# aszepieniec/stark-brainfuck

Measured on AMD Instinct MI355X. Metric: goldilocks_ntt_field_elements_per_sec, higher is better.
Workload: dtype u64 (mod 2^64-2^32+1)

## Files before the change

stark_brainfuck_amd/csrc/air.hip:

```cpp
#include <algorithm>
#include <cstddef>
#include <vector>

#include "air_eval.hpp"
#include "lazy.hpp"
#include "runtime.hpp"

namespace bfs {

struct RandomizerValues {
    u64 v[64];
};

__global__ void __launch_bounds__(256) poly_evaluate_partial_kernel(const u64* coeffs, u64 stride, u64 h, u64 point, u64* partial, u32 first) {
    __shared__ u64 part[256];
    const u64* f = coeffs + (u64)(first + blockIdx.y) * stride;
    const u32 t = threadIdx.x;
    const u64 T = (u64)gridDim.x * 256, g = (u64)blockIdx.x * 256 + t;
    u64 acc = 0;
    if (g < h) {
        const u64 step = gl_pow(point, T);
        u64 k = g + (h - 1 - g) / T * T;
        for (;; k -= T) {
            acc = gl_add(gl_mul(acc, step), f[k]);
// ... 26 lines not shown
    __shared__ u64 part[256];
    const u64* f = coeffs + (u64)blockIdx.y * stride;
    u64 acc = 0;
    for (u64 j = (u64)blockIdx.x * 256 + threadIdx.x; j < len; j += (u64)gridDim.x * 256)
        if (f[j] != 0) acc |= j ? (j & (0 - j)) : (1ull << 63);
    part[threadIdx.x] = acc;
    __syncthreads();
    for (u32 s = 128; s > 0; s >>= 1) {
        if (threadIdx.x < s) part[threadIdx.x] |= part[threadIdx.x + s];
        __syncthreads();
    }
    if (threadIdx.x == 0 && part[0]) atomicOr((unsigned long long*)(out + blockIdx.y), (unsigned long long)part[0]);
}

struct AirArgs {
    const u64* base;
    const u64* ext;
    u64* out;
    u64 n;
    u64 first, count;
    u64 unit_distance;
    u64 height;
    u32 log_height;
    u64 omicron_inv;
    u64 offset;
    const u64* w_lo;
    const u64* w_hi;
    u32 lo_bits;
    Xfe ch[11];
    Xfe tm[5];
    Xfe pr[1];
};

struct LdsNextBase {
    const u64* p;
    __device__ __forceinline__ u64 operator[](int k) const { return p[k * 256]; }
};
struct LdsNextExt {
    const u64* p;
    __device__ __forceinline__ Xfe operator[](int k) const { return Xfe{{p[(3 * k) * 256], p[(3 * k + 1) * 256], p[(3 * k + 2) * 256]}}; }
};

struct Zerofiers {
    u64 boundary, transition, terminal;
    __device__ __forceinline__ Zerofiers(const AirArgs& a, u64 x) {
        const u64 za = gl_sub(x, 1), xo = gl_sub(x, a.omicron_inv);
        u64 zc = 1;
        if (a.height != 0) {
            u64 xh = x;
            for (u32 s = 0; s < a.log_height; ++s) xh = gl_sqr(xh);
            zc = gl_sub(xh, 1);
        }
        const u64 ab = gl_mul(za, xo);
        const u64 iabc = gl_inv(gl_mul(ab, zc));
        const u64 iab = gl_mul(iabc, zc);
        boundary = gl_mul(iab, xo);
        terminal = gl_mul(iab, za);
        transition = a.height != 0 ? gl_mul(xo, gl_mul(iabc, ab)) : 0;
    }
    __device__ __forceinline__ Zerofiers(const AirArgs& a, u64 x, u64 inv_x_minus_1, u64 inv_x_minus_omicron_inv, u64 inv_xh_minus_1) {
        boundary = inv_x_minus_1;
        terminal = inv_x_minus_omicron_inv;
        transition = a.height != 0 ? gl_mul(gl_sub(x, a.omicron_inv), inv_xh_minus_1) : 0;
    }
    template <int TABLE, int Q>
    __device__ __forceinline__ u64 of() const {
        typedef AirShape<TABLE> S;
        return Q < S::NB ? boundary : (Q < S::NB + S::NT ? transition : terminal);
    }
};

template <int TABLE>
struct QuotientStore {
    u64* out;
    u64 n, i;
    Zerofiers z;
    template <int Q> __device__ __forceinline__ void put(const Xfe& v) {
// ... 94 lines not shown
    static constexpr int kind(int k) { return k < NC ? 0 : (k - NC < S::NB ? 1 : (k - NC < S::NB + S::NT ? 2 : 3)); }
    static constexpr bool continues_run(int k) {
        if (k == 0 || kind(k) != kind(k - 1)) return false;
        return kind(k) == 0 ? true : q_degree(k - NC) == q_degree(k - 1 - NC);
    }
    static constexpr int words(int k) { return 2 * (is_ext(k) ? LAZY_W_EXT : LAZY_W_BASE); }
    static constexpr int offset(int k) {
        int o = 0;
        for (int j = 0; j < k; ++j) o += words(j);
        return o;
    }
    static constexpr int NW = offset(NTERM);
};

template <int TABLE>
struct CombineTerms {
    u64 w[CombineLayout<TABLE>::NW];
    u32 shift[(CombineLayout<TABLE>::NTERM + 1) & ~1];
};

template <int TABLE>
struct AirCombineArgs {
    AirArgs a;
    const u64* randomizer;
    Xfe w0;
    u64* acc;
    const u64 *inv_boundary, *inv_terminal, *inv_transition;
    CombineTerms<TABLE> terms;
};

template <int TABLE, bool GROUPED>
struct CombineSink {
    typedef CombineLayout<TABLE> Lay;
    const AirArgs& a;
    const CombineTerms<TABLE>& T;
    u64 i;
    Zerofiers z;
    Xfe acc;
    LazyX sa, sb;

    __device__ __forceinline__ u64 omega_pow(int k) const {
        return tw_pow(a.w_lo, a.w_hi, a.lo_bits, (i * T.shift[k]) & (a.n - 1));
    }
    template <int K> __device__ __forceinline__ void close_run() {
        lazyx_mac_scale(sa, lazyx_reduce(sb), omega_pow(K));
        sb = lazyx_zero();
    }
    template <int KIND> __device__ __forceinline__ void close_kind() {
        const Xfe kind_sum = lazyx_reduce(sa);
        sa = lazyx_zero();
        if constexpr (KIND == 0) acc = xfe_add(acc, kind_sum);
        else acc = xfe_add(acc, xfe_scale(kind_sum, KIND == 1 ? z.boundary : (KIND == 2 ? z.transition : z.terminal)));
    }
    template <int K> __device__ __forceinline__ void open() {
        if constexpr (K > 0) {
            constexpr bool new_kind = Lay::kind(K) != Lay::kind(K - 1);
            if constexpr (new_kind || !GROUPED || !Lay::continues_run(K)) close_run<K - 1>();
            if constexpr (new_kind) close_kind<Lay::kind(K - 1)>();
        }
    }
    template <int K> __device__ __forceinline__ void term_base(u64 v) {
        static_assert(!Lay::is_ext(K), "layout and generated code disagree");
        open<K>();
        lazyx_mac_base(sa, T.w + Lay::offset(K), v);
        lazyx_mac_base(sb, T.w + Lay::offset(K) + LAZY_W_BASE, v);
    }
    template <int K> __device__ __forceinline__ void term_ext(const Xfe& v) {
        static_assert(Lay::is_ext(K), "layout and generated code disagree");
        open<K>();
        lazyx_mac_ext(sa, T.w + Lay::offset(K), v);
        lazyx_mac_ext(sb, T.w + Lay::offset(K) + LAZY_W_EXT, v);
    }
    __device__ __forceinline__ void finish() {
        close_run<Lay::NTERM - 1>();
        close_kind<Lay::kind(Lay::NTERM - 1)>();
    }
    template <int Q> __device__ __forceinline__ void put(const Xfe& v) { term_ext<Lay::NC + Q>(v); }
    template <int Q> __device__ __forceinline__ void put_base(u64 v) { term_base<Lay::NC + Q>(v); }
};

template <int TABLE, int C, class Sink>
__device__ __forceinline__ void combine_columns(Sink& sink, const u64* bc, const Xfe* xc) {
    typedef AirShape<TABLE> S;
    if constexpr (C < S::BW) { sink.template term_base<C>(bc[C]); combine_columns<TABLE, C + 1>(sink, bc, xc); }
    else if constexpr (C < S::BW + S::XW) { sink.template term_ext<C>(xc[C - S::BW]); combine_columns<TABLE, C + 1>(sink, bc, xc); }
}

#ifndef BFS_COMBINE_WAVES
#define BFS_COMBINE_WAVES 3, 3, 4, 4, 4
#endif
#ifndef BFS_COMBINE_LDS_NEXT
#define BFS_COMBINE_LDS_NEXT 1
#endif
constexpr int combine_waves(int table) {
    constexpr int w[5] = {BFS_COMBINE_WAVES};
    return w[table];
}
template <int TABLE, bool GROUPED>
__global__ void __launch_bounds__(256, combine_waves(TABLE)) air_combine_kernel(const AirCombineArgs<TABLE> A) {
    typedef AirShape<TABLE> S;
    __shared__ CombineTerms<TABLE> T;
    {
        const u64* karg = (const u64*)__builtin_amdgcn_kernarg_segment_ptr();
        constexpr u32 first = offsetof(AirCombineArgs<TABLE>, terms) / 8, words = sizeof(CombineTerms<TABLE>) / 8;
        static_assert(offsetof(AirCombineArgs<TABLE>, terms) % 8 == 0 && sizeof(CombineTerms<TABLE>) % 8 == 0, "staged as 64-bit words");
        u64* dst = reinterpret_cast<u64*>(&T);
        for (u32 k = threadIdx.x; k < words; k += 256) dst[k] = karg[first + k];
    }
    __syncthreads();
    const AirArgs& a = A.a;
    const u64 i = a.first + (u64)blockIdx.x * blockDim.x + threadIdx.x;
    if (i < a.first + a.count) {
        u64 j = i + a.unit_distance;
        if (j >= a.n) j -= a.n;
        constexpr bool LDS_NEXT = ((BFS_COMBINE_LDS_NEXT) >> TABLE) & 1;
        __shared__ u64 next_row[LDS_NEXT ? (S::BW + 3 * S::XW) * 256 : 1];
        u64 bc[S::BW], bn[LDS_NEXT ? 1 : S::BW];
        Xfe xc[S::XW], xn[LDS_NEXT ? 1 : S::XW];
#pragma unroll
        for (int c = 0; c < S::BW; ++c) {
            bc[c] = a.base[(u64)c * a.n + i];
            if constexpr (LDS_NEXT) next_row[c * 256 + threadIdx.x] = a.base[(u64)c * a.n + j];
            else bn[c] = a.base[(u64)c * a.n + j];
        }
#pragma unroll
        for (int c = 0; c < S::XW; ++c)
#pragma unroll
            for (int l = 0; l < 3; ++l) {
                xc[c].c[l] = a.ext[(u64)(3 * c + l) * a.n + i];
                if constexpr (LDS_NEXT) next_row[(S::BW + 3 * c + l) * 256 + threadIdx.x] = a.ext[(u64)(3 * c + l) * a.n + j];
                else xn[c].c[l] = a.ext[(u64)(3 * c + l) * a.n + j];
            }
        Xfe acc;
        if (A.randomizer) acc = xfe_mul(A.w0, Xfe{{A.randomizer[i], A.randomizer[a.n + i], A.randomizer[2 * a.n + i]}});
        else acc = Xfe{{A.acc[i], A.acc[a.n + i], A.acc[2 * a.n + i]}};
        const u64 x = gl_mul(a.offset, tw_pow(a.w_lo, a.w_hi, a.lo_bits, i));
        CombineSink<TABLE, GROUPED> sink{a, T, i,
                                         A.inv_boundary ? Zerofiers(a, x, A.inv_boundary[i], A.inv_terminal[i], a.height != 0 ? A.inv_transition[i] : 0)
                                                        : Zerofiers(a, x),
                                         acc, lazyx_zero(), lazyx_zero()};
        combine_columns<TABLE, 0>(sink, bc, xc);
        if constexpr (LDS_NEXT) air_eval<TABLE>(bc, LdsNextBase{next_row + threadIdx.x}, xc, LdsNextExt{next_row + S::BW * 256 + threadIdx.x}, a, sink);
        else air_eval<TABLE>(bc, (const u64*)bn, xc, (const Xfe*)xn, a, sink);
        sink.finish();
        A.acc[i] = sink.acc.c[0];
        A.acc[a.n + i] = sink.acc.c[1];
        A.acc[2 * a.n + i] = sink.acc.c[2];
    }
}

__global__ void difference_combine_kernel(const u64* lhs, const u64* rhs, u64* acc, u64 n, u64 offset, const u64* w_lo, const u64* w_hi,
                                          u32 lo_bits, CombW w, const u64* inv_x_minus_1, u64 first, u64 count) {
    for (u64 i = first + (u64)blockIdx.x * blockDim.x + threadIdx.x; i < first + count; i += (u64)gridDim.x * blockDim.x) {
        const u64 z = inv_x_minus_1 ? inv_x_minus_1[i] : gl_inv(gl_sub(gl_mul(offset, tw_pow(w_lo, w_hi, lo_bits, i)), 1));
        const u64 xs = gl_mul(w.offset_pow, tw_pow(w_lo, w_hi, lo_bits, (i * w.shift) & (n - 1)));
        const Xfe weight = xfe_add(w.wa, xfe_scale(w.wb, xs));
        Xfe q;
#pragma unroll
        for (int l = 0; l < 3; ++l) q.c[l] = gl_mul(gl_sub(lhs[(u64)l * n + i], rhs[(u64)l * n + i]), z);
        const Xfe r = xfe_add(Xfe{{acc[i], acc[n + i], acc[2 * n + i]}}, xfe_mul(weight, q));
        acc[i] = r.c[0];
        acc[n + i] = r.c[1];
        acc[2 * n + i] = r.c[2];
    }
}

__global__ void difference_quotient_kernel(const u64* lhs, const u64* rhs, u64* out, u64 n, u64 offset, const u64* w_lo, const u64* w_hi, u32 lo_bits) {
    for (u64 i = (u64)blockIdx.x * blockDim.x + threadIdx.x; i < n; i += (u64)gridDim.x * blockDim.x) {
        const u64 x = gl_mul(offset, tw_pow(w_lo, w_hi, lo_bits, i));
        const u64 z = gl_inv(gl_sub(x, 1));
#pragma unroll
        for (int l = 0; l < 3; ++l) out[(u64)l * n + i] = gl_mul(gl_sub(lhs[(u64)l * n + i], rhs[(u64)l * n + i]), z);
    }
}

struct CombSrc {
    const u64* ptr;
    u32 is_ext, pad;
    u64 shift;
    Xfe wa, wb;
// ... 346 lines not shown
```

stark_brainfuck_amd/csrc/air_eval.hpp:

```cpp
#pragma once
#include "air_generated.hpp"

namespace bfs {

template <int TABLE> struct AirShape;
template <> struct AirShape<0> { static constexpr int BW = airgen::PROCESSOR_BASE_WIDTH, XW = airgen::PROCESSOR_EXT_WIDTH, NB = airgen::PROCESSOR_NUM_BOUNDARY, NT = airgen::PROCESSOR_NUM_TRANSITION, NZ = airgen::PROCESSOR_NUM_TERMINAL; };
template <> struct AirShape<1> { static constexpr int BW = airgen::INSTRUCTION_BASE_WIDTH, XW = airgen::INSTRUCTION_EXT_WIDTH, NB = airgen::INSTRUCTION_NUM_BOUNDARY, NT = airgen::INSTRUCTION_NUM_TRANSITION, NZ = airgen::INSTRUCTION_NUM_TERMINAL; };
template <> struct AirShape<2> { static constexpr int BW = airgen::MEMORY_BASE_WIDTH, XW = airgen::MEMORY_EXT_WIDTH, NB = airgen::MEMORY_NUM_BOUNDARY, NT = airgen::MEMORY_NUM_TRANSITION, NZ = airgen::MEMORY_NUM_TERMINAL; };
template <> struct AirShape<3> { static constexpr int BW = airgen::INPUT_BASE_WIDTH, XW = airgen::INPUT_EXT_WIDTH, NB = airgen::INPUT_NUM_BOUNDARY, NT = airgen::INPUT_NUM_TRANSITION, NZ = airgen::INPUT_NUM_TERMINAL; };
template <> struct AirShape<4> { static constexpr int BW = airgen::OUTPUT_BASE_WIDTH, XW = airgen::OUTPUT_EXT_WIDTH, NB = airgen::OUTPUT_NUM_BOUNDARY, NT = airgen::OUTPUT_NUM_TRANSITION, NZ = airgen::OUTPUT_NUM_TERMINAL; };

template <int TABLE, class Sink, class BN, class XN, class Args>
__device__ __forceinline__ void air_eval(const u64* bc, BN bn, const Xfe* xc, XN xn, const Args& a, Sink& sink) {
    if constexpr (TABLE == 0) airgen::air_processor(bc, bn, xc, xn, a.ch, a.tm, a.pr, sink);
    else if constexpr (TABLE == 1) airgen::air_instruction(bc, bn, xc, xn, a.ch, a.tm, a.pr, sink);
    else if constexpr (TABLE == 2) airgen::air_memory(bc, bn, xc, xn, a.ch, a.tm, a.pr, sink);
    else if constexpr (TABLE == 3) airgen::air_input(bc, bn, xc, xn, a.ch, a.tm, a.pr, sink);
    else airgen::air_output(bc, bn, xc, xn, a.ch, a.tm, a.pr, sink);
}

}
```

stark_brainfuck_amd/csrc/air_generated.hpp:

```cpp
#pragma once
#include "gl.hpp"

namespace bfs {
namespace airgen {

struct ArraySink {
    Xfe* out;
    template <int I> BFS_HD void put(const Xfe& v) { out[I] = v; }
    template <int I> BFS_HD void put_base(u64 v) { out[I] = xfe_lift(v); }
};

constexpr int PROCESSOR_BASE_WIDTH = 7, PROCESSOR_EXT_WIDTH = 4, PROCESSOR_NUM_BOUNDARY = 7, PROCESSOR_NUM_TRANSITION = 10, PROCESSOR_NUM_TERMINAL = 4;
constexpr bool PROCESSOR_Q_EXT[] = {false, false, false, false, false, true, true, false, false, false, false, false, false, true, true, true, true, true, true, true, true};
constexpr unsigned char PROCESSOR_Q_DEGREE[] = {1, 1, 1, 1, 1, 1, 1, 11, 9, 9, 1, 3, 3, 9, 9, 9, 9, 1, 9, 1, 1};
template <class Sink, class BN = const u64*, class XN = const Xfe*>
BFS_HD void air_processor(const u64* bc, BN bn, const Xfe* xc, XN xn, const Xfe* ch, const Xfe* tm, const Xfe* pr, Sink& sink) {
    sink.template put_base<0>(bc[0]);
    sink.template put_base<1>(bc[1]);
    sink.template put_base<2>(bc[4]);
    sink.template put_base<3>(bc[5]);
    sink.template put_base<4>(bc[6]);
    sink.template put<5>(xc[2]);
    sink.template put<6>(xc[3]);
    const u64 t0 = gl_sub(bc[2], 93ULL);
    const u64 t1 = gl_sub(bc[2], 60ULL);
    const u64 t2 = gl_mul(t0, t1);
    const u64 t3 = gl_sub(bc[2], 62ULL);
    const u64 t4 = gl_mul(t2, t3);
    const u64 t5 = gl_sub(bc[2], 44ULL);
    const u64 t6 = gl_mul(t4, t5);
    const u64 t7 = gl_sub(bc[2], 46ULL);
    const u64 t8 = gl_mul(t6, t7);
    const u64 t9 = gl_sub(bc[2], 43ULL);
    const u64 t10 = gl_mul(t8, t9);
    const u64 t11 = gl_sub(bc[2], 45ULL);
    const u64 t12 = gl_mul(t10, t11);
    const u64 t13 = gl_sub(bn[1], bc[1]);
    const u64 t14 = gl_sub(t13, 2ULL);
    const u64 t15 = gl_mul(bc[5], t14);
    const u64 t16 = gl_mul(bc[5], bc[6]);
    const u64 t17 = gl_sub(t16, 1ULL);
    const u64 t18 = gl_sub(bn[1], bc[3]);
    const u64 t19 = gl_mul(t17, t18);
    const u64 t20 = gl_add(t15, t19);
    const u64 t21 = gl_mul(t20, bc[2]);
    const u64 t22 = gl_mul(t12, t21);
    const u64 t23 = gl_sub(bc[2], 91ULL);
// ... 127 lines not shown
    const Xfe t143 = xfe_scale(t142, bc[2]);
    const Xfe t144 = xfe_sub(xn[2], xc[2]);
    const u64 t145 = gl_sub(44ULL, bc[2]);
    const Xfe t146 = xfe_scale(t144, t145);
    const Xfe t147 = xfe_add(t143, t146);
    sink.template put<15>(t147);
    const Xfe t148 = xfe_mul(xc[3], ch[9]);
    const Xfe t149 = xfe_sub(xn[3], t148);
    const Xfe t150 = xfe_sub_base(t149, bc[5]);
    const Xfe t151 = xfe_scale(t150, t68);
    const Xfe t152 = xfe_scale(t151, bc[2]);
    const Xfe t153 = xfe_sub(xn[3], xc[3]);
    const u64 t154 = gl_sub(46ULL, bc[2]);
    const Xfe t155 = xfe_scale(t153, t154);
    const Xfe t156 = xfe_add(t152, t155);
    sink.template put<16>(t156);
    const Xfe t157 = xfe_sub(tm[0], xc[0]);
    sink.template put<17>(t157);
    const Xfe t158 = xfe_sub(tm[1], t133);
    const Xfe t159 = xfe_scale(t158, bc[2]);
    const Xfe t160 = xfe_sub(tm[1], xc[1]);
    const Xfe t161 = xfe_scale(t160, t123);
    const Xfe t162 = xfe_add(t159, t161);
    sink.template put<18>(t162);
    const Xfe t163 = xfe_sub(tm[2], xc[2]);
    sink.template put<19>(t163);
    const Xfe t164 = xfe_sub(tm[3], xc[3]);
    sink.template put<20>(t164);
}
BFS_HD void air_processor_values(const u64* bc, const u64* bn, const Xfe* xc, const Xfe* xn, const Xfe* ch, const Xfe* tm, const Xfe* pr, Xfe* out) {
    ArraySink sink{out};
    air_processor(bc, bn, xc, xn, ch, tm, pr, sink);
}

constexpr int INSTRUCTION_BASE_WIDTH = 3, INSTRUCTION_EXT_WIDTH = 2, INSTRUCTION_NUM_BOUNDARY = 2, INSTRUCTION_NUM_TRANSITION = 6, INSTRUCTION_NUM_TERMINAL = 2;
constexpr bool INSTRUCTION_Q_EXT[] = {false, true, false, false, false, false, true, true, true, true};
constexpr unsigned char INSTRUCTION_Q_DEGREE[] = {1, 1, 2, 2, 2, 2, 9, 2, 1, 1};
template <class Sink, class BN = const u64*, class XN = const Xfe*>
BFS_HD void air_instruction(const u64* bc, BN bn, const Xfe* xc, XN xn, const Xfe* ch, const Xfe* tm, const Xfe* pr, Sink& sink) {
    sink.template put_base<0>(bc[0]);
    const Xfe t0 = xfe_scale(ch[0], bc[0]);
    const Xfe t1 = xfe_sub(xc[1], t0);
    const Xfe t2 = xfe_scale(ch[1], bc[1]);
    const Xfe t3 = xfe_sub(t1, t2);
    const Xfe t4 = xfe_scale(ch[2], bc[2]);
    const Xfe t5 = xfe_sub(t3, t4);
    sink.template put<1>(t5);
    const u64 t6 = gl_sub(bn[0], bc[0]);
    const u64 t7 = gl_sub(t6, 1ULL);
    const u64 t8 = gl_mul(t7, t6);
    sink.template put_base<2>(t8);
    const u64 t9 = gl_sub(bc[2], bn[1]);
    const u64 t10 = gl_mul(t6, t9);
    sink.template put_base<3>(t10);
    const u64 t11 = gl_sub(bn[1], bc[1]);
    const u64 t12 = gl_mul(t7, t11);
    sink.template put_base<4>(t12);
    const u64 t13 = gl_sub(bn[2], bc[2]);
    const u64 t14 = gl_mul(t7, t13);
    sink.template put_base<5>(t14);
    const Xfe t15 = xfe_scale(ch[0], bn[0]);
    const Xfe t16 = xfe_sub(ch[6], t15);
    const Xfe t17 = xfe_scale(ch[1], bn[1]);
    const Xfe t18 = xfe_sub(t16, t17);
    const Xfe t19 = xfe_scale(ch[2], bn[2]);
    const Xfe t20 = xfe_sub(t18, t19);
    const Xfe t21 = xfe_mul(xc[0], t20);
    const Xfe t22 = xfe_sub(t21, xn[0]);
    const Xfe t23 = xfe_scale(t22, bc[1]);
    const u64 t24 = gl_add(bc[0], 1ULL);
// ... 10 lines not shown
    const u64 t35 = gl_mul(t33, t34);
    const u64 t36 = gl_sub(bc[1], 45ULL);
    const u64 t37 = gl_mul(t35, t36);
    const u64 t38 = gl_sub(bc[1], 44ULL);
    const u64 t39 = gl_mul(t37, t38);
    const u64 t40 = gl_sub(bc[1], 46ULL);
    const u64 t41 = gl_mul(t39, t40);
    const Xfe t42 = xfe_sub(xc[0], xn[0]);
    const Xfe t43 = xfe_scale(t42, t41);
    const Xfe t44 = xfe_add(t26, t43);
    const u64 t45 = gl_sub(bc[0], bn[0]);
    const Xfe t46 = xfe_scale(t42, t45);
    const Xfe t47 = xfe_add(t44, t46);
    sink.template put<6>(t47);
    const Xfe t48 = xfe_mul(xc[1], ch[10]);
    const Xfe t49 = xfe_add(t48, t15);
    const Xfe t50 = xfe_add(t49, t17);
    const Xfe t51 = xfe_add(t50, t19);
    const Xfe t52 = xfe_sub(t51, xn[1]);
    const Xfe t53 = xfe_scale(t52, t6);
    const Xfe t54 = xfe_sub(xc[1], xn[1]);
    const Xfe t55 = xfe_scale(t54, t7);
    const Xfe t56 = xfe_add(t53, t55);
    sink.template put<7>(t56);
    const Xfe t57 = xfe_sub(xc[0], tm[0]);
    sink.template put<8>(t57);
    const Xfe t58 = xfe_sub(xc[1], tm[4]);
    sink.template put<9>(t58);
}
BFS_HD void air_instruction_values(const u64* bc, const u64* bn, const Xfe* xc, const Xfe* xn, const Xfe* ch, const Xfe* tm, const Xfe* pr, Xfe* out) {
    ArraySink sink{out};
    air_instruction(bc, bn, xc, xn, ch, tm, pr, sink);
}

constexpr int MEMORY_BASE_WIDTH = 4, MEMORY_EXT_WIDTH = 1, MEMORY_NUM_BOUNDARY = 3, MEMORY_NUM_TRANSITION = 7, MEMORY_NUM_TERMINAL = 1;
constexpr bool MEMORY_Q_EXT[] = {false, false, false, false, false, false, false, false, false, true, true};
constexpr unsigned char MEMORY_Q_DEGREE[] = {1, 1, 1, 2, 2, 2, 2, 2, 2, 3, 3};
template <class Sink, class BN = const u64*, class XN = const Xfe*>
BFS_HD void air_memory(const u64* bc, BN bn, const Xfe* xc, XN xn, const Xfe* ch, const Xfe* tm, const Xfe* pr, Sink& sink) {
    sink.template put_base<0>(bc[0]);
    sink.template put_base<1>(bc[1]);
    sink.template put_base<2>(bc[2]);
    const u64 t0 = gl_sub(bn[1], bc[1]);
    const u64 t1 = gl_sub(t0, 1ULL);
    const u64 t2 = gl_mul(t1, t0);
    sink.template put_base<3>(t2);
    const u64 t3 = gl_mul(t0, bn[2]);
    sink.template put_base<4>(t3);
    const u64 t4 = gl_sub(bn[3], 1ULL);
    const u64 t5 = gl_mul(t4, bn[3]);
    sink.template put_base<5>(t5);
    const u64 t6 = gl_mul(bc[3], t0);
    sink.template put_base<6>(t6);
    const u64 t7 = gl_sub(bn[2], bc[2]);
    const u64 t8 = gl_mul(bc[3], t7);
    sink.template put_base<7>(t8);
    const u64 t9 = gl_sub(bn[1], 1ULL);
    const u64 t10 = gl_sub(t9, bc[1]);
    const u64 t11 = gl_sub(bn[0], 1ULL);
    const u64 t12 = gl_sub(t11, bc[0]);
    const u64 t13 = gl_mul(t10, t12);
    sink.template put_base<8>(t13);
    const Xfe t14 = xfe_scale(ch[3], bc[0]);
    const Xfe t15 = xfe_sub(ch[7], t14);
    const Xfe t16 = xfe_scale(ch[4], bc[1]);
    const Xfe t17 = xfe_sub(t15, t16);
    const Xfe t18 = xfe_scale(ch[5], bc[2]);
    const Xfe t19 = xfe_sub(t17, t18);
    const Xfe t20 = xfe_mul(xc[0], t19);
    const Xfe t21 = xfe_sub(t20, xn[0]);
    const u64 t22 = gl_sub(1ULL, bc[3]);
    const Xfe t23 = xfe_scale(t21, t22);
    const Xfe t24 = xfe_sub(xc[0], xn[0]);
    const Xfe t25 = xfe_scale(t24, bc[3]);
    const Xfe t26 = xfe_add(t23, t25);
    sink.template put<9>(t26);
    const Xfe t27 = xfe_sub(t20, tm[1]);
    const Xfe t28 = xfe_scale(t27, t22);
    const Xfe t29 = xfe_sub(xc[0], tm[1]);
    const Xfe t30 = xfe_scale(t29, bc[3]);
    const Xfe t31 = xfe_add(t28, t30);
    sink.template put<10>(t31);
}
BFS_HD void air_memory_values(const u64* bc, const u64* bn, const Xfe* xc, const Xfe* xn, const Xfe* ch, const Xfe* tm, const Xfe* pr, Xfe* out) {
    ArraySink sink{out};
    air_memory(bc, bn, xc, xn, ch, tm, pr, sink);
}

constexpr int INPUT_BASE_WIDTH = 1, INPUT_EXT_WIDTH = 1, INPUT_NUM_BOUNDARY = 1, INPUT_NUM_TRANSITION = 1, INPUT_NUM_TERMINAL = 1;
constexpr bool INPUT_Q_EXT[] = {true, true, true};
constexpr unsigned char INPUT_Q_DEGREE[] = {1, 1, 1};
template <class Sink, class BN = const u64*, class XN = const Xfe*>
BFS_HD void air_input(const u64* bc, BN bn, const Xfe* xc, XN xn, const Xfe* ch, const Xfe* tm, const Xfe* pr, Sink& sink) {
    const Xfe t0 = xfe_sub_base(xc[0], bc[0]);
    sink.template put<0>(t0);
    const Xfe t1 = xfe_mul(xc[0], ch[8]);
    const Xfe t2 = xfe_add_base(t1, bn[0]);
    const Xfe t3 = xfe_sub(t2, xn[0]);
    sink.template put<1>(t3);
    const Xfe t4 = xfe_mul(tm[2], pr[0]);
    const Xfe t5 = xfe_sub(xc[0], t4);
    sink.template put<2>(t5);
}
BFS_HD void air_input_values(const u64* bc, const u64* bn, const Xfe* xc, const Xfe* xn, const Xfe* ch, const Xfe* tm, const Xfe* pr, Xfe* out) {
    ArraySink sink{out};
    air_input(bc, bn, xc, xn, ch, tm, pr, sink);
}

constexpr int OUTPUT_BASE_WIDTH = 1, OUTPUT_EXT_WIDTH = 1, OUTPUT_NUM_BOUNDARY = 1, OUTPUT_NUM_TRANSITION = 1, OUTPUT_NUM_TERMINAL = 1;
constexpr bool OUTPUT_Q_EXT[] = {true, true, true};
constexpr unsigned char OUTPUT_Q_DEGREE[] = {1, 1, 1};
template <class Sink, class BN = const u64*, class XN = const Xfe*>
BFS_HD void air_output(const u64* bc, BN bn, const Xfe* xc, XN xn, const Xfe* ch, const Xfe* tm, const Xfe* pr, Sink& sink) {
    const Xfe t0 = xfe_sub_base(xc[0], bc[0]);
    sink.template put<0>(t0);
    const Xfe t1 = xfe_mul(xc[0], ch[9]);
    const Xfe t2 = xfe_add_base(t1, bn[0]);
    const Xfe t3 = xfe_sub(t2, xn[0]);
    sink.template put<1>(t3);
    const Xfe t4 = xfe_mul(tm[3], pr[0]);
    const Xfe t5 = xfe_sub(xc[0], t4);
    sink.template put<2>(t5);
}
BFS_HD void air_output_values(const u64* bc, const u64* bn, const Xfe* xc, const Xfe* xn, const Xfe* ch, const Xfe* tm, const Xfe* pr, Xfe* out) {
    ArraySink sink{out};
    air_output(bc, bn, xc, xn, ch, tm, pr, sink);
}

}
}
```

Before: 102.5 billion.

## Stage processor AIR combine to cut register pressure and shrink next-row LDS

The processor table's constraint combination is restructured into a staged form. Each constraint kind is flushed to the global accumulator as soon as it is complete, and current-row extension columns are refetched from memory instead of being held in registers. Challenge constants are moved into LDS, and sched barriers fence the stages. Next-row LDS staging now covers only the columns the constraints actually use, and the processor kernel's occupancy hint rises from 3 to 4 waves. The aim is lower VGPR pressure and higher occupancy, paid for with extra global read-modify-writes of the accumulator, repeated zerofier work and refetched loads.

```diff
diff --git a/stark_brainfuck_amd/csrc/air.hip b/stark_brainfuck_amd/csrc/air.hip
--- a/stark_brainfuck_amd/csrc/air.hip
+++ b/stark_brainfuck_amd/csrc/air.hip
@@ -82,17 +82,42 @@
     Xfe pr[1];
 };
 
+constexpr int next_slot(unsigned mask, int k) { return __builtin_popcount(mask & ((1u << k) - 1)); }
+template <unsigned MASK>
 struct LdsNextBase {
     const u64* p;
-    __device__ __forceinline__ u64 operator[](int k) const { return p[k * 256]; }
-};
+    __device__ __forceinline__ u64 operator[](int k) const { return p[next_slot(MASK, k) * 256]; }
+};
+template <unsigned MASK>
 struct LdsNextExt {
     const u64* p;
-    __device__ __forceinline__ Xfe operator[](int k) const { return Xfe{{p[(3 * k) * 256], p[(3 * k + 1) * 256], p[(3 * k + 2) * 256]}}; }
-};
+    __device__ __forceinline__ Xfe operator[](int k) const {
+        const int s = 3 * next_slot(MASK, k);
+        return Xfe{{p[s * 256], p[(s + 1) * 256], p[(s + 2) * 256]}};
+    }
+};
+
+struct RefetchedExt {
+    const u64* p;
+    u64 n;
+    __device__ __forceinline__ Xfe operator[](int k) const {
+        const u64* q = p + (u64)(3 * k) * n;
+        asm volatile("" : "+v"(q));
+        return Xfe{{q[0], q[n], q[2 * n]}};
+    }
+};
+struct AirConstants {
+    Xfe ch[11];
+    Xfe tm[5];
+    Xfe pr[1];
+};
+static_assert(offsetof(AirArgs, ch) % 8 == 0 && offsetof(AirArgs, tm) - offsetof(AirArgs, ch) == offsetof(AirConstants, tm) &&
+              offsetof(AirArgs, pr) - offsetof(AirArgs, ch) == offsetof(AirConstants, pr) && sizeof(AirArgs) - offsetof(AirArgs, ch) == sizeof(AirConstants),
+              "AirConstants is the tail of AirArgs");
 
 struct Zerofiers {
     u64 boundary, transition, terminal;
+    __device__ __forceinline__ Zerofiers() : boundary(0), transition(0), terminal(0) {}
     __device__ __forceinline__ Zerofiers(const AirArgs& a, u64 x) {
         const u64 za = gl_sub(x, 1), xo = gl_sub(x, a.omicron_inv);
         u64 zc = 1;
@@ -253,13 +278,32 @@
 template <int TABLE, bool GROUPED>
 struct CombineSink {
     typedef CombineLayout<TABLE> Lay;
+    const AirCombineArgs<TABLE>& A;
     const AirArgs& a;
     const CombineTerms<TABLE>& T;
     u64 i;
+    Xfe acc;
     Zerofiers z;
-    Xfe acc;
+    bool fresh;
     LazyX sa, sb;
 
+    __device__ __forceinline__ Xfe accumulator() const {
+        if (fresh && A.randomizer) return xfe_mul(A.w0, Xfe{{A.randomizer[i], A.randomizer[a.n + i], A.randomizer[2 * a.n + i]}});
+        return Xfe{{A.acc[i], A.acc[a.n + i], A.acc[2 * a.n + i]}};
+    }
+    __device__ __forceinline__ Zerofiers zerofiers() const {
+        const u64 x = gl_mul(a.offset, tw_pow(a.w_lo, a.w_hi, a.lo_bits, i));
+        return A.inv_boundary ? Zerofiers(a, x, A.inv_boundary[i], A.inv_terminal[i], a.height != 0 ? A.inv_transition[i] : 0) : Zerofiers(a, x);
+    }
+    __device__ __forceinline__ void store(const Xfe& r) {
+        A.acc[i] = r.c[0];
+        A.acc[a.n + i] = r.c[1];
+        A.acc[2 * a.n + i] = r.c[2];
+    }
+    __device__ __forceinline__ void flush(const Xfe& share) {
+        store(xfe_add(accumulator(), share));
+        fresh = false;
+    }
     __device__ __forceinline__ u64 omega_pow(int k) const {
         return tw_pow(a.w_lo, a.w_hi, a.lo_bits, (i * T.shift[k]) & (a.n - 1));
     }
@@ -267,17 +311,39 @@
         lazyx_mac_scale(sa, lazyx_reduce(sb), omega_pow(K));
         sb = lazyx_zero();
     }
+    template <int KIND> __device__ __forceinline__ u64 zerofier_inverse() const {
+        if constexpr (!AirShape<TABLE>::STAGED) return KIND == 1 ? z.boundary : (KIND == 2 ? z.transition : z.terminal);
+        if (A.inv_boundary) {
+            if constexpr (KIND == 1) return A.inv_boundary[i];
+            else if constexpr (KIND == 3) return A.inv_terminal[i];
+            else return a.height != 0 ? gl_mul(gl_sub(gl_mul(a.offset, tw_pow(a.w_lo, a.w_hi, a.lo_bits, i)), a.omicron_inv), A.inv_transition[i]) : 0;
+        }
+        const Zerofiers here(a, gl_mul(a.offset, tw_pow(a.w_lo, a.w_hi, a.lo_bits, i)));
+        return KIND == 1 ? here.boundary : (KIND == 2 ? here.transition : here.terminal);
+    }
     template <int KIND> __device__ __forceinline__ void close_kind() {
         const Xfe kind_sum = lazyx_reduce(sa);
         sa = lazyx_zero();
-        if constexpr (KIND == 0) acc = xfe_add(acc, kind_sum);
-        else acc = xfe_add(acc, xfe_scale(kind_sum, KIND == 1 ? z.boundary : (KIND == 2 ? z.transition : z.terminal)));
+        Xfe share = kind_sum;
+        if constexpr (KIND != 0) share = xfe_scale(kind_sum, zerofier_inverse<KIND>());
+        if constexpr (AirShape<TABLE>::STAGED) flush(share);
+        else acc = xfe_add(acc, share);
     }
     template <int K> __device__ __forceinline__ void open() {
-        if constexpr (K > 0) {
-            constexpr bool new_kind = Lay::kind(K) != Lay::kind(K - 1);
-            if constexpr (new_kind || !GROUPED || !Lay::continues_run(K)) close_run<K - 1>();
-            if constexpr (new_kind) close_kind<Lay::kind(K - 1)>();
+        constexpr bool staged = AirShape<TABLE>::STAGED, first_of_kind = K == 0 || Lay::kind(K) != Lay::kind(K - 1);
+        if constexpr (staged) __builtin_amdgcn_sched_barrier(0);
+        if constexpr (!first_of_kind) {
+            if constexpr (!GROUPED || !Lay::continues_run(K)) close_run<K - 1>();
+        } else if constexpr (!staged && K > 0) {
+            close_run<K - 1>();
+            close_kind<Lay::kind(K - 1)>();
+        }
+    }
+    template <int K> __device__ __forceinline__ void close() {
+        constexpr bool last_of_kind = K == Lay::NTERM - 1 || Lay::kind(K + 1) != Lay::kind(K);
+        if constexpr (last_of_kind && (AirShape<TABLE>::STAGED || K == Lay::NTERM - 1)) {
+            close_run<K>();
+            close_kind<Lay::kind(K)>();
         }
     }
     template <int K> __device__ __forceinline__ void term_base(u64 v) {
@@ -285,30 +351,29 @@
         open<K>();
         lazyx_mac_base(sa, T.w + Lay::offset(K), v);
         lazyx_mac_base(sb, T.w + Lay::offset(K) + LAZY_W_BASE, v);
+        close<K>();
     }
     template <int K> __device__ __forceinline__ void term_ext(const Xfe& v) {
         static_assert(Lay::is_ext(K), "layout and generated code disagree");
         open<K>();
         lazyx_mac_ext(sa, T.w + Lay::offset(K), v);
         lazyx_mac_ext(sb, T.w + Lay::offset(K) + LAZY_W_EXT, v);
-    }
-    __device__ __forceinline__ void finish() {
-        close_run<Lay::NTERM - 1>();
-        close_kind<Lay::kind(Lay::NTERM - 1)>();
-    }
+        close<K>();
+    }
+    __device__ __forceinline__ void fence() { __builtin_amdgcn_sched_barrier(0); }
     template <int Q> __device__ __forceinline__ void put(const Xfe& v) { term_ext<Lay::NC + Q>(v); }
     template <int Q> __device__ __forceinline__ void put_base(u64 v) { term_base<Lay::NC + Q>(v); }
 };
 
-template <int TABLE, int C, class Sink>
-__device__ __forceinline__ void combine_columns(Sink& sink, const u64* bc, const Xfe* xc) {
+template <int TABLE, int C, class Sink, class XC>
+__device__ __forceinline__ void combine_columns(Sink& sink, const u64* bc, XC xc) {
     typedef AirShape<TABLE> S;
     if constexpr (C < S::BW) { sink.template term_base<C>(bc[C]); combine_columns<TABLE, C + 1>(sink, bc, xc); }
     else if constexpr (C < S::BW + S::XW) { sink.template term_ext<C>(xc[C - S::BW]); combine_columns<TABLE, C + 1>(sink, bc, xc); }
 }
 
 #ifndef BFS_COMBINE_WAVES
-#define BFS_COMBINE_WAVES 3, 3, 4, 4, 4
+#define BFS_COMBINE_WAVES 4, 3, 4, 4, 4
 #endif
 #ifndef BFS_COMBINE_LDS_NEXT
 #define BFS_COMBINE_LDS_NEXT 1
@@ -328,6 +393,12 @@
         u64* dst = reinterpret_cast<u64*>(&T);
         for (u32 k = threadIdx.x; k < words; k += 256) dst[k] = karg[first + k];
     }
+    __shared__ u64 constants[S::STAGED ? sizeof(AirConstants) / 8 : 1];
+    if constexpr (S::STAGED) {
+        const u64* karg = (const u64*)__builtin_amdgcn_kernarg_segment_ptr();
+        static_assert(offsetof(AirCombineArgs<TABLE>, a) == 0 && sizeof(AirConstants) / 8 <= 256, "one word per thread");
+        if (threadIdx.x < sizeof(AirConstants) / 8) constants[threadIdx.x] = karg[offsetof(AirArgs, ch) / 8 + threadIdx.x];
+    }
     __syncthreads();
     const AirArgs& a = A.a;
     const u64 i = a.first + (u64)blockIdx.x * blockDim.x + threadIdx.x;
@@ -335,38 +406,44 @@
         u64 j = i + a.unit_distance;
         if (j >= a.n) j -= a.n;
         constexpr bool LDS_NEXT = ((BFS_COMBINE_LDS_NEXT) >> TABLE) & 1;
-        __shared__ u64 next_row[LDS_NEXT ? (S::BW + 3 * S::XW) * 256 : 1];
+        constexpr int NEXT_WORDS = __builtin_popcount(S::NEXT_BASE) + 3 * __builtin_popcount(S::NEXT_EXT), NEXT_EXT_AT = __builtin_popcount(S::NEXT_BASE);
+        __shared__ u64 next_row[LDS_NEXT ? NEXT_WORDS * 256 : 1];
         u64 bc[S::BW], bn[LDS_NEXT ? 1 : S::BW];
-        Xfe xc[S::XW], xn[LDS_NEXT ? 1 : S::XW];
+        Xfe xc[S::STAGED ? 1 : S::XW], xn[LDS_NEXT ? 1 : S::XW];
 #pragma unroll
         for (int c = 0; c < S::BW; ++c) {
             bc[c] = a.base[(u64)c * a.n + i];
-            if constexpr (LDS_NEXT) next_row[c * 256 + threadIdx.x] = a.base[(u64)c * a.n + j];
-            else bn[c] = a.base[(u64)c * a.n + j];
+            if constexpr (LDS_NEXT) {
+                if ((S::NEXT_BASE >> c) & 1) next_row[next_slot(S::NEXT_BASE, c) * 256 + threadIdx.x] = a.base[(u64)c * a.n + j];
+            } else bn[c] = a.base[(u64)c * a.n + j];
         }
 #pragma unroll
         for (int c = 0; c < S::XW; ++c)
 #pragma unroll
             for (int l = 0; l < 3; ++l) {
-                xc[c].c[l] = a.ext[(u64)(3 * c + l) * a.n + i];
-                if constexpr (LDS_NEXT) next_row[(S::BW + 3 * c + l) * 256 + threadIdx.x] = a.ext[(u64)(3 * c + l) * a.n + j];
-                else xn[c].c[l] = a.ext[(u64)(3 * c + l) * a.n + j];
+                if constexpr (!S::STAGED) xc[c].c[l] = a.ext[(u64)(3 * c + l) * a.n + i];
+                if constexpr (LDS_NEXT) {
+                    if ((S::NEXT_EXT >> c) & 1) next_row[(NEXT_EXT_AT + 3 * next_slot(S::NEXT_EXT, c) + l) * 256 + threadIdx.x] = a.ext[(u64)(3 * c + l) * a.n + j];
+                } else xn[c].c[l] = a.ext[(u64)(3 * c + l) * a.n + j];
             }
-        Xfe acc;
-        if (A.randomizer) acc = xfe_mul(A.w0, Xfe{{A.randomizer[i], A.randomizer[a.n + i], A.randomizer[2 * a.n + i]}});
-        else acc = Xfe{{A.acc[i], A.acc[a.n + i], A.acc[2 * a.n + i]}};
-        const u64 x = gl_mul(a.offset, tw_pow(a.w_lo, a.w_hi, a.lo_bits, i));
-        CombineSink<TABLE, GROUPED> sink{a, T, i,
-                                         A.inv_boundary ? Zerofiers(a, x, A.inv_boundary[i], A.inv_terminal[i], a.height != 0 ? A.inv_transition[i] : 0)
-                                                        : Zerofiers(a, x),
-                                         acc, lazyx_zero(), lazyx_zero()};
-        combine_columns<TABLE, 0>(sink, bc, xc);
-        if constexpr (LDS_NEXT) air_eval<TABLE>(bc, LdsNextBase{next_row + threadIdx.x}, xc, LdsNextExt{next_row + S::BW * 256 + threadIdx.x}, a, sink);
-        else air_eval<TABLE>(bc, (const u64*)bn, xc, (const Xfe*)xn, a, sink);
-        sink.finish();
-        A.acc[i] = sink.acc.c[0];
-        A.acc[a.n + i] = sink.acc.c[1];
-        A.acc[2 * a.n + i] = sink.acc.c[2];
+        CombineSink<TABLE, GROUPED> sink{A, a, T, i, Xfe{{0, 0, 0}}, Zerofiers(), true, lazyx_zero(), lazyx_zero()};
+        if constexpr (!S::STAGED) {
+            sink.acc = sink.accumulator();
+            sink.z = sink.zerofiers();
+        }
+        if constexpr (S::STAGED) {
+            static_assert(LDS_NEXT, "the staged tables keep their next row in LDS");
+            const RefetchedExt xr{a.ext + i, a.n};
+            air_eval_staged<TABLE>(bc, LdsNextBase<S::NEXT_BASE>{next_row + threadIdx.x}, xr, LdsNextExt<S::NEXT_EXT>{next_row + NEXT_EXT_AT * 256 + threadIdx.x},
+                                   *reinterpret_cast<const AirConstants*>(constants), sink);
+            combine_columns<TABLE, 0>(sink, bc, xr);
+        } else {
+            combine_columns<TABLE, 0>(sink, bc, (const Xfe*)xc);
+            if constexpr (LDS_NEXT)
+                air_eval<TABLE>(bc, LdsNextBase<S::NEXT_BASE>{next_row + threadIdx.x}, xc, LdsNextExt<S::NEXT_EXT>{next_row + NEXT_EXT_AT * 256 + threadIdx.x}, a, sink);
+            else air_eval<TABLE>(bc, (const u64*)bn, xc, (const Xfe*)xn, a, sink);
+        }
+        if constexpr (!S::STAGED) sink.store(sink.acc);
     }
 }
 
diff --git a/stark_brainfuck_amd/csrc/air_eval.hpp b/stark_brainfuck_amd/csrc/air_eval.hpp
--- a/stark_brainfuck_amd/csrc/air_eval.hpp
+++ b/stark_brainfuck_amd/csrc/air_eval.hpp
@@ -4,11 +4,11 @@
 namespace bfs {
 
 template <int TABLE> struct AirShape;
-template <> struct AirShape<0> { static constexpr int BW = airgen::PROCESSOR_BASE_WIDTH, XW = airgen::PROCESSOR_EXT_WIDTH, NB = airgen::PROCESSOR_NUM_BOUNDARY, NT = airgen::PROCESSOR_NUM_TRANSITION, NZ = airgen::PROCESSOR_NUM_TERMINAL; };
-template <> struct AirShape<1> { static constexpr int BW = airgen::INSTRUCTION_BASE_WIDTH, XW = airgen::INSTRUCTION_EXT_WIDTH, NB = airgen::INSTRUCTION_NUM_BOUNDARY, NT = airgen::INSTRUCTION_NUM_TRANSITION, NZ = airgen::INSTRUCTION_NUM_TERMINAL; };
-template <> struct AirShape<2> { static constexpr int BW = airgen::MEMORY_BASE_WIDTH, XW = airgen::MEMORY_EXT_WIDTH, NB = airgen::MEMORY_NUM_BOUNDARY, NT = airgen::MEMORY_NUM_TRANSITION, NZ = airgen::MEMORY_NUM_TERMINAL; };
-template <> struct AirShape<3> { static constexpr int BW = airgen::INPUT_BASE_WIDTH, XW = airgen::INPUT_EXT_WIDTH, NB = airgen::INPUT_NUM_BOUNDARY, NT = airgen::INPUT_NUM_TRANSITION, NZ = airgen::INPUT_NUM_TERMINAL; };
-template <> struct AirShape<4> { static constexpr int BW = airgen::OUTPUT_BASE_WIDTH, XW = airgen::OUTPUT_EXT_WIDTH, NB = airgen::OUTPUT_NUM_BOUNDARY, NT = airgen::OUTPUT_NUM_TRANSITION, NZ = airgen::OUTPUT_NUM_TERMINAL; };
+template <> struct AirShape<0> { static constexpr int BW = airgen::PROCESSOR_BASE_WIDTH, XW = airgen::PROCESSOR_EXT_WIDTH, NB = airgen::PROCESSOR_NUM_BOUNDARY, NT = airgen::PROCESSOR_NUM_TRANSITION, NZ = airgen::PROCESSOR_NUM_TERMINAL; static constexpr unsigned NEXT_BASE = airgen::PROCESSOR_NEXT_BASE_USED, NEXT_EXT = airgen::PROCESSOR_NEXT_EXT_USED; static constexpr bool STAGED = airgen::PROCESSOR_STAGED; };
+template <> struct AirShape<1> { static constexpr int BW = airgen::INSTRUCTION_BASE_WIDTH, XW = airgen::INSTRUCTION_EXT_WIDTH, NB = airgen::INSTRUCTION_NUM_BOUNDARY, NT = airgen::INSTRUCTION_NUM_TRANSITION, NZ = airgen::INSTRUCTION_NUM_TERMINAL; static constexpr unsigned NEXT_BASE = airgen::INSTRUCTION_NEXT_BASE_USED, NEXT_EXT = airgen::INSTRUCTION_NEXT_EXT_USED; static constexpr bool STAGED = airgen::INSTRUCTION_STAGED; };
+template <> struct AirShape<2> { static constexpr int BW = airgen::MEMORY_BASE_WIDTH, XW = airgen::MEMORY_EXT_WIDTH, NB = airgen::MEMORY_NUM_BOUNDARY, NT = airgen::MEMORY_NUM_TRANSITION, NZ = airgen::MEMORY_NUM_TERMINAL; static constexpr unsigned NEXT_BASE = airgen::MEMORY_NEXT_BASE_USED, NEXT_EXT = airgen::MEMORY_NEXT_EXT_USED; static constexpr bool STAGED = airgen::MEMORY_STAGED; };
+template <> struct AirShape<3> { static constexpr int BW = airgen::INPUT_BASE_WIDTH, XW = airgen::INPUT_EXT_WIDTH, NB = airgen::INPUT_NUM_BOUNDARY, NT = airgen::INPUT_NUM_TRANSITION, NZ = airgen::INPUT_NUM_TERMINAL; static constexpr unsigned NEXT_BASE = airgen::INPUT_NEXT_BASE_USED, NEXT_EXT = airgen::INPUT_NEXT_EXT_USED; static constexpr bool STAGED = airgen::INPUT_STAGED; };
+template <> struct AirShape<4> { static constexpr int BW = airgen::OUTPUT_BASE_WIDTH, XW = airgen::OUTPUT_EXT_WIDTH, NB = airgen::OUTPUT_NUM_BOUNDARY, NT = airgen::OUTPUT_NUM_TRANSITION, NZ = airgen::OUTPUT_NUM_TERMINAL; static constexpr unsigned NEXT_BASE = airgen::OUTPUT_NEXT_BASE_USED, NEXT_EXT = airgen::OUTPUT_NEXT_EXT_USED; static constexpr bool STAGED = airgen::OUTPUT_STAGED; };
 
 template <int TABLE, class Sink, class BN, class XN, class Args>
 __device__ __forceinline__ void air_eval(const u64* bc, BN bn, const Xfe* xc, XN xn, const Args& a, Sink& sink) {
@@ -19,4 +19,10 @@
     else airgen::air_output(bc, bn, xc, xn, a.ch, a.tm, a.pr, sink);
 }
 
+template <int TABLE, class Sink, class BN, class XC, class XN, class Args>
+__device__ __forceinline__ void air_eval_staged(const u64* bc, BN bn, XC xc, XN xn, const Args& a, Sink& sink) {
+    static_assert(TABLE == 0 && AirShape<TABLE>::STAGED, "no staged constraint code for this table");
+    airgen::air_processor_staged(bc, bn, xc, xn, a.ch, a.tm, a.pr, sink);
 }
+
+}
diff --git a/stark_brainfuck_amd/csrc/air_generated.hpp b/stark_brainfuck_amd/csrc/air_generated.hpp
--- a/stark_brainfuck_amd/csrc/air_generated.hpp
+++ b/stark_brainfuck_amd/csrc/air_generated.hpp
@@ -8,11 +8,13 @@
     Xfe* out;
     template <int I> BFS_HD void put(const Xfe& v) { out[I] = v; }
     template <int I> BFS_HD void put_base(u64 v) { out[I] = xfe_lift(v); }
+    BFS_HD void fence() {}
 };
 
 constexpr int PROCESSOR_BASE_WIDTH = 7, PROCESSOR_EXT_WIDTH = 4, PROCESSOR_NUM_BOUNDARY = 7, PROCESSOR_NUM_TRANSITION = 10, PROCESSOR_NUM_TERMINAL = 4;
 constexpr bool PROCESSOR_Q_EXT[] = {false, false, false, false, false, true, true, false, false, false, false, false, false, true, true, true, true, true, true, true, true};
 constexpr unsigned char PROCESSOR_Q_DEGREE[] = {1, 1, 1, 1, 1, 1, 1, 11, 9, 9, 1, 3, 3, 9, 9, 9, 9, 1, 9, 1, 1};
+constexpr unsigned PROCESSOR_NEXT_BASE_USED = 0x33, PROCESSOR_NEXT_EXT_USED = 0xf;
 template <class Sink, class BN = const u64*, class XN = const Xfe*>
 BFS_HD void air_processor(const u64* bc, BN bn, const Xfe* xc, XN xn, const Xfe* ch, const Xfe* tm, const Xfe* pr, Sink& sink) {
     sink.template put_base<0>(bc[0]);
@@ -206,10 +208,206 @@
     ArraySink sink{out};
     air_processor(bc, bn, xc, xn, ch, tm, pr, sink);
 }
+constexpr bool PROCESSOR_STAGED = true;
+template <class Sink, class BN = const u64*, class XC = const Xfe*, class XN = const Xfe*>
+BFS_HD void air_processor_staged(const u64* bc, BN bn, XC xc, XN xn, const Xfe* ch, const Xfe* tm, const Xfe* pr, Sink& sink) {
+    const u64 t0 = gl_sub(bc[2], 93ULL);
+    const u64 t1 = gl_sub(bc[2], 60ULL);
+    const u64 t2 = gl_mul(t0, t1);
+    const u64 t3 = gl_sub(bc[2], 62ULL);
+    const u64 t4 = gl_mul(t2, t3);
+    const u64 t5 = gl_sub(bc[2], 44ULL);
+    const u64 t6 = gl_mul(t4, t5);
+    const u64 t7 = gl_sub(bc[2], 46ULL);
+    const u64 t8 = gl_mul(t6, t7);
+    const u64 t9 = gl_sub(bc[2], 43ULL);
+    const u64 t10 = gl_mul(t8, t9);
+    const u64 t11 = gl_sub(bc[2], 45ULL);
+    const u64 t12 = gl_mul(t10, t11);
+    const u64 t13 = gl_sub(bn[1], bc[1]);
+    const u64 t14 = gl_sub(t13, 2ULL);
+    const u64 t15 = gl_mul(bc[5], t14);
+    const u64 t16 = gl_mul(bc[5], bc[6]);
+    const u64 t17 = gl_sub(t16, 1ULL);
+    const u64 t18 = gl_sub(bn[1], bc[3]);
+    const u64 t19 = gl_mul(t17, t18);
+    const u64 t20 = gl_add(t15, t19);
+    const u64 t21 = gl_mul(t20, bc[2]);
+    const u64 t22 = gl_mul(t12, t21);
+    const u64 t23 = gl_sub(bc[2], 91ULL);
+    const u64 t24 = gl_mul(t23, t1);
+    const u64 t25 = gl_mul(t24, t3);
+    const u64 t26 = gl_mul(t25, t5);
+    const u64 t27 = gl_mul(t26, t7);
+    const u64 t28 = gl_mul(t27, t9);
+    const u64 t29 = gl_mul(t28, t11);
+    const u64 t30 = gl_mul(t17, t14);
+    const u64 t31 = gl_mul(bc[5], t18);
+    const u64 t32 = gl_add(t30, t31);
+    const u64 t33 = gl_mul(t32, bc[2]);
+    const u64 t34 = gl_mul(t29, t33);
+    const u64 t35 = gl_add(t22, t34);
+    const u64 t36 = gl_mul(t23, t0);
+    const u64 t37 = gl_mul(t36, t3);
+    const u64 t38 = gl_mul(t37, t5);
+    const u64 t39 = gl_mul(t38, t7);
+    const u64 t40 = gl_mul(t39, t9);
+    const u64 t41 = gl_mul(t40, t11);
+    const u64 t42 = gl_sub(t13, 1ULL);
+    const u64 t43 = gl_mul(t42, bc[2]);
+    const u64 t44 = gl_mul(t41, t43);
+    const u64 t45 = gl_add(t35, t44);
+    const u64 t46 = gl_mul(t36, t1);
+    const u64 t47 = gl_mul(t46, t5);
+    const u64 t48 = gl_mul(t47, t7);
+    const u64 t49 = gl_mul(t48, t9);
+    const u64 t50 = gl_mul(t49, t11);
+    const u64 t51 = gl_mul(t50, t43);
+    const u64 t52 = gl_add(t45, t51);
+    const u64 t53 = gl_mul(t46, t3);
+    const u64 t54 = gl_mul(t53, t5);
+    const u64 t55 = gl_mul(t54, t7);
+    const u64 t56 = gl_mul(t55, t11);
+    const u64 t57 = gl_mul(t56, t43);
+    const u64 t58 = gl_add(t52, t57);
+    const u64 t59 = gl_mul(t55, t9);
+    const u64 t60 = gl_mul(t59, t43);
+    const u64 t61 = gl_add(t58, t60);
+    const u64 t62 = gl_mul(t53, t7);
+    const u64 t63 = gl_mul(t62, t9);
+    const u64 t64 = gl_mul(t63, t11);
+    const u64 t65 = gl_mul(t64, t43);
+    const u64 t66 = gl_add(t61, t65);
+    const u64 t67 = gl_mul(t54, t9);
+    const u64 t68 = gl_mul(t67, t11);
+    const u64 t69 = gl_mul(t68, t43);
+    const u64 t70 = gl_add(t66, t69);
+    const u64 t71 = gl_sub(bn[4], bc[4]);
+    const u64 t72 = gl_mul(t71, bc[2]);
+    const u64 t73 = gl_mul(t12, t72);
+    const u64 t74 = gl_mul(t29, t72);
+    const u64 t75 = gl_add(t73, t74);
+    const u64 t76 = gl_add(t71, 1ULL);
+    const u64 t77 = gl_mul(t76, bc[2]);
+    const u64 t78 = gl_mul(t41, t77);
+    const u64 t79 = gl_add(t75, t78);
+    const u64 t80 = gl_sub(t71, 1ULL);
+    const u64 t81 = gl_mul(t80, bc[2]);
+    const u64 t82 = gl_mul(t50, t81);
+    const u64 t83 = gl_add(t79, t82);
+    const u64 t84 = gl_mul(t56, t72);
+    const u64 t85 = gl_add(t83, t84);
+    const u64 t86 = gl_mul(t59, t72);
+    const u64 t87 = gl_add(t85, t86);
+    const u64 t88 = gl_mul(t64, t72);
+    const u64 t89 = gl_add(t87, t88);
+    const u64 t90 = gl_mul(t68, t72);
+    const u64 t91 = gl_add(t89, t90);
+    const u64 t92 = gl_sub(bn[5], bc[5]);
+    const u64 t93 = gl_mul(t92, bc[2]);
+    const u64 t94 = gl_mul(t12, t93);
+    const u64 t95 = gl_mul(t29, t93);
+    const u64 t96 = gl_add(t94, t95);
+    const u64 t97 = gl_sub(t92, 1ULL);
+    const u64 t98 = gl_mul(t97, bc[2]);
+    const u64 t99 = gl_mul(t56, t98);
+    const u64 t100 = gl_add(t96, t99);
+    const u64 t101 = gl_add(t92, 1ULL);
+    const u64 t102 = gl_mul(t101, bc[2]);
+    const u64 t103 = gl_mul(t59, t102);
+    const u64 t104 = gl_add(t100, t103);
+    const u64 t105 = gl_mul(t68, t93);
+    const u64 t106 = gl_add(t104, t105);
+    const u64 t107 = gl_sub(bn[0], bc[0]);
+    const u64 t108 = gl_sub(t107, 1ULL);
+    const u64 t109 = gl_mul(bc[5], t17);
+    const u64 t110 = gl_mul(bc[6], t17);
+    const u64 t120 = gl_mul(t53, t9);
+    const u64 t121 = gl_mul(t120, t11);
+    const u64 t122 = gl_mul(t121, t5);
+    const u64 t123 = gl_mul(t122, t7);
+    const u64 t145 = gl_sub(44ULL, bc[2]);
+    const u64 t154 = gl_sub(46ULL, bc[2]);
+    sink.fence();
+    sink.template put_base<7>(t70);
+    sink.template put_base<8>(t91);
+    sink.template put_base<9>(t106);
+    sink.template put_base<10>(t108);
+    sink.template put_base<11>(t109);
+    sink.template put_base<12>(t110);
+    const Xfe t111 = xfe_scale(ch[0], bc[1]);
+    const Xfe t112 = xfe_sub(ch[6], t111);
+    const Xfe t113 = xfe_scale(ch[1], bc[2]);
+    const Xfe t114 = xfe_sub(t112, t113);
+    const Xfe t115 = xfe_scale(ch[2], bc[3]);
+    const Xfe t116 = xfe_sub(t114, t115);
+    const Xfe t117 = xfe_mul(xc[0], t116);
+    const Xfe t118 = xfe_sub(t117, xn[0]);
+    const Xfe t119 = xfe_scale(t118, bc[2]);
+    const Xfe t124 = xfe_sub(xc[0], xn[0]);
+    const Xfe t125 = xfe_scale(t124, t123);
+    const Xfe t126 = xfe_add(t119, t125);
+    sink.template put<13>(t126);
+    const Xfe t127 = xfe_scale(ch[3], bc[0]);
+    const Xfe t128 = xfe_sub(ch[7], t127);
+    const Xfe t129 = xfe_scale(ch[4], bc[4]);
+    const Xfe t130 = xfe_sub(t128, t129);
+    const Xfe t131 = xfe_scale(ch[5], bc[5]);
+    const Xfe t132 = xfe_sub(t130, t131);
+    const Xfe t133 = xfe_mul(xc[1], t132);
+    const Xfe t134 = xfe_sub(t133, xn[1]);
+    const Xfe t135 = xfe_scale(t134, bc[2]);
+    const Xfe t136 = xfe_sub(xc[1], xn[1]);
+    const Xfe t137 = xfe_scale(t136, t123);
+    const Xfe t138 = xfe_add(t135, t137);
+    sink.template put<14>(t138);
+    const Xfe t139 = xfe_mul(xc[2], ch[8]);
+    const Xfe t140 = xfe_sub(xn[2], t139);
+    const Xfe t141 = xfe_sub_base(t140, bn[5]);
+    const Xfe t142 = xfe_scale(t141, t64);
+    const Xfe t143 = xfe_scale(t142, bc[2]);
+    const Xfe t144 = xfe_sub(xn[2], xc[2]);
+    const Xfe t146 = xfe_scale(t144, t145);
+    const Xfe t147 = xfe_add(t143, t146);
+    sink.template put<15>(t147);
+    const Xfe t148 = xfe_mul(xc[3], ch[9]);
+    const Xfe t149 = xfe_sub(xn[3], t148);
+    const Xfe t150 = xfe_sub_base(t149, bc[5]);
+    const Xfe t151 = xfe_scale(t150, t68);
+    const Xfe t152 = xfe_scale(t151, bc[2]);
+    const Xfe t153 = xfe_sub(xn[3], xc[3]);
+    const Xfe t155 = xfe_scale(t153, t154);
+    const Xfe t156 = xfe_add(t152, t155);
+    sink.template put<16>(t156);
+    sink.template put_base<0>(bc[0]);
+    sink.template put_base<1>(bc[1]);
+    sink.template put_base<2>(bc[4]);
+    sink.template put_base<3>(bc[5]);
+    sink.template put_base<4>(bc[6]);
+    sink.template put<5>(xc[2]);
+    sink.template put<6>(xc[3]);
+    const Xfe t157 = xfe_sub(tm[0], xc[0]);
+    sink.template put<17>(t157);
+    const Xfe t158 = xfe_sub(tm[1], t133);
+    const Xfe t159 = xfe_scale(t158, bc[2]);
+    const Xfe t160 = xfe_sub(tm[1], xc[1]);
+    const Xfe t161 = xfe_scale(t160, t123);
+    const Xfe t162 = xfe_add(t159, t161);
+    sink.template put<18>(t162);
+    const Xfe t163 = xfe_sub(tm[2], xc[2]);
+    sink.template put<19>(t163);
+    const Xfe t164 = xfe_sub(tm[3], xc[3]);
+    sink.template put<20>(t164);
+}
+BFS_HD void air_processor_staged_values(const u64* bc, const u64* bn, const Xfe* xc, const Xfe* xn, const Xfe* ch, const Xfe* tm, const Xfe* pr, Xfe* out) {
+    ArraySink sink{out};
+    air_processor_staged(bc, bn, xc, xn, ch, tm, pr, sink);
+}
 
 constexpr int INSTRUCTION_BASE_WIDTH = 3, INSTRUCTION_EXT_WIDTH = 2, INSTRUCTION_NUM_BOUNDARY = 2, INSTRUCTION_NUM_TRANSITION = 6, INSTRUCTION_NUM_TERMINAL = 2;
 constexpr bool INSTRUCTION_Q_EXT[] = {false, true, false, false, false, false, true, true, true, true};
 constexpr unsigned char INSTRUCTION_Q_DEGREE[] = {1, 1, 2, 2, 2, 2, 9, 2, 1, 1};
+constexpr unsigned INSTRUCTION_NEXT_BASE_USED = 0x7, INSTRUCTION_NEXT_EXT_USED = 0x3;
 template <class Sink, class BN = const u64*, class XN = const Xfe*>
 BFS_HD void air_instruction(const u64* bc, BN bn, const Xfe* xc, XN xn, const Xfe* ch, const Xfe* tm, const Xfe* pr, Sink& sink) {
     sink.template put_base<0>(bc[0]);
@@ -286,10 +484,12 @@
     ArraySink sink{out};
     air_instruction(bc, bn, xc, xn, ch, tm, pr, sink);
 }
+constexpr bool INSTRUCTION_STAGED = false;
 
 constexpr int MEMORY_BASE_WIDTH = 4, MEMORY_EXT_WIDTH = 1, MEMORY_NUM_BOUNDARY = 3, MEMORY_NUM_TRANSITION = 7, MEMORY_NUM_TERMINAL = 1;
 constexpr bool MEMORY_Q_EXT[] = {false, false, false, false, false, false, false, false, false, true, true};
 constexpr unsigned char MEMORY_Q_DEGREE[] = {1, 1, 1, 2, 2, 2, 2, 2, 2, 3, 3};
+constexpr unsigned MEMORY_NEXT_BASE_USED = 0xf, MEMORY_NEXT_EXT_USED = 0x1;
 template <class Sink, class BN = const u64*, class XN = const Xfe*>
 BFS_HD void air_memory(const u64* bc, BN bn, const Xfe* xc, XN xn, const Xfe* ch, const Xfe* tm, const Xfe* pr, Sink& sink) {
     sink.template put_base<0>(bc[0]);
@@ -340,10 +540,12 @@
     ArraySink sink{out};
     air_memory(bc, bn, xc, xn, ch, tm, pr, sink);
 }
+constexpr bool MEMORY_STAGED = false;
 
 constexpr int INPUT_BASE_WIDTH = 1, INPUT_EXT_WIDTH = 1, INPUT_NUM_BOUNDARY = 1, INPUT_NUM_TRANSITION = 1, INPUT_NUM_TERMINAL = 1;
 constexpr bool INPUT_Q_EXT[] = {true, true, true};
 constexpr unsigned char INPUT_Q_DEGREE[] = {1, 1, 1};
+constexpr unsigned INPUT_NEXT_BASE_USED = 0x1, INPUT_NEXT_EXT_USED = 0x1;
 template <class Sink, class BN = const u64*, class XN = const Xfe*>
 BFS_HD void air_input(const u64* bc, BN bn, const Xfe* xc, XN xn, const Xfe* ch, const Xfe* tm, const Xfe* pr, Sink& sink) {
     const Xfe t0 = xfe_sub_base(xc[0], bc[0]);
@@ -360,10 +562,12 @@
     ArraySink sink{out};
     air_input(bc, bn, xc, xn, ch, tm, pr, sink);
 }
+constexpr bool INPUT_STAGED = false;
 
 constexpr int OUTPUT_BASE_WIDTH = 1, OUTPUT_EXT_WIDTH = 1, OUTPUT_NUM_BOUNDARY = 1, OUTPUT_NUM_TRANSITION = 1, OUTPUT_NUM_TERMINAL = 1;
 constexpr bool OUTPUT_Q_EXT[] = {true, true, true};
 constexpr unsigned char OUTPUT_Q_DEGREE[] = {1, 1, 1};
+constexpr unsigned OUTPUT_NEXT_BASE_USED = 0x1, OUTPUT_NEXT_EXT_USED = 0x1;
 template <class Sink, class BN = const u64*, class XN = const Xfe*>
 BFS_HD void air_output(const u64* bc, BN bn, const Xfe* xc, XN xn, const Xfe* ch, const Xfe* tm, const Xfe* pr, Sink& sink) {
     const Xfe t0 = xfe_sub_base(xc[0], bc[0]);
@@ -380,6 +584,7 @@
     ArraySink sink{out};
     air_output(bc, bn, xc, xn, ch, tm, pr, sink);
 }
-
-}
-}
+constexpr bool OUTPUT_STAGED = false;
+
+}
+}
```

Result: no change. 102.5 billion, median of 2 (-0.0%).
